# LockedFlysher/optimal_control_problem

Hardware: AMD Instinct MI355X
Metric: QP solves/sec (batched OSQP-ADMM, N=20) (higher is better)
Workload: dtype f64

## Files before the change

optimal_control_problem_amd/csrc/kernel_oc_split.hpp:

```cpp
#pragma once

constexpr int OC_PENDING = 100, OC_PENDING_NONCVX = 101;
template <int NW>
struct OcLds {
  double *X, *Q, *R, *Z, *Y, *W, *RB, *RED;
  int *octab, *co;
};
template <int NW, bool SETUP = false>
__device__ __forceinline__ OcLds<NW> oc_lds(double *lds, const DevPlan &pl, const DevRes &rs, const DevOc &oc) {
  OcLds<NW> L;
  L.X = lds + rs.stage; L.Q = L.X + pl.npad; L.R = SETUP ? L.Q : L.Q + pl.npad;
  double *rend = L.R + pl.npad + rs.rext;
  L.Z = rend; L.Y = L.Z + (SETUP ? oc.zpad : pl.mpad); L.W = L.Y + (SETUP ? pl.npad : pl.mpad);
  L.RB = L.W + pl.mpad; L.RED = L.RB + 16 * NW + 16;
  L.octab = reinterpret_cast<int *>(L.RED + 16 * NW) + 8;
  L.co = L.octab + ((oc.o_pos + 1) & ~1);
  return L;
}
__device__ __forceinline__ int oc_wave_role4(double *lds, int wid, const int lane, const int no_remap) {
  const unsigned hw = __builtin_amdgcn_s_getreg((31 << 11) | 4), la = __builtin_amdgcn_s_getreg((31 << 11) | 6);
  const int simd = (hw >> 4) & 3, slot = (la & 0xff) != 0;
  int *xs = reinterpret_cast<int *>(lds);
  if (lane == 0) xs[wid] = simd;
  bsync<4>();
// ... 65 lines not shown
    cx.rho = uni(io.info[4L * b + 3]);
    cx.c = 1.0; cx.cinv = 1.0;
    const bool okr = factorize_res<NW, (HUB ? 2 : 1), false>(cx, &oc, L.octab, lds);
    if (tid == 0) io.status[b] = okr ? OC_PENDING : OC_PENDING_NONCVX;
    return;
  }
  double c = 1.0;
  int refactor = 1, prev_status = MPCQP_UNSOLVED;
  const bool reuse = REUSE && io.reuse;
  if (reuse) {
    prev_status = io.status[b];
    c = io.cscale[b];
    for (int t = tid; t < npad; t += NT) { if (pl.perm[t] < 0) Qs[t] = 0.0; cx.R[t] = Dg[t]; }
    bsync<NW>();
    for (int j = tid; j < n; j += NT) { const int t = pl.pos[j]; Qs[t] = inq[j] * (c * cx.R[t]); }
    double chg[1] = {0.0};
    for (int i = tid; i < mpad; i += NT) {
      const double ei = Eg[i];
      const double nl = i < m ? ei * fmax(inl[i], -Q_INFTY) : 0.0, nu = i < m ? ei * fmin(inu[i], Q_INFTY) : 0.0;
      if (i < m) {
        const double ol = lb[i], ou = ub[i];
        const int oc_ = (ol < -Q_INFTY * Q_MIN_SCALING && ou > Q_INFTY * Q_MIN_SCALING) ? 0 : (ou - ol < Q_RHO_TOL ? 2 : 1);
        const int nc = (nl < -Q_INFTY * Q_MIN_SCALING && nu > Q_INFTY * Q_MIN_SCALING) ? 0 : (nu - nl < Q_RHO_TOL ? 2 : 1);
        if (oc_ != nc) chg[0] = 1.0;
      }
      lb[i] = nl; ub[i] = nu;
    }
    block_combine<NW, 1, 0>(chg, cx.RED, wid, lane);
    refactor = chg[0] != 0.0;
    c = uni(c); cx.c = c; cx.cinv = uni(1.0 / c);
    bsync<NW>();
  } else {
    const bool a_lds = oc.a_lds, p_lds = oc.p_lds;
    auto scale_phase = [&](double *sA, double *sP, auto iA, auto iP) __attribute__((always_inline)) {
    auto gather8 = [&](const int *__restrict__ src, const double *__restrict__ in, double *dst, const long entries) __attribute__((always_inline)) {
      long e = tid;
      for (; e + 7L * NT < entries; e += 8L * NT) {
        int sr[8]; double v[8];
#pragma unroll
        for (int u = 0; u < 8; u++) sr[u] = src[e + (long)u * NT];
#pragma unroll
        for (int u = 0; u < 8; u++) v[u] = in[max(sr[u], 0)];
#pragma unroll
        for (int u = 0; u < 8; u++) dst[e + (long)u * NT] = sr[u] >= 0 ? v[u] : 0.0;
      }
      for (; e < entries; e += NT) { const int sr = src[e]; dst[e] = sr >= 0 ? in[sr] : 0.0; }
    };
    gather8(pl.A.src, inA, sA, pl.A.entries);
    gather8(pl.P.src, inP, sP, pl.P.entries);
    if constexpr (sizeof(*iA) == 2) { for (long e = tid; e < pl.A.entries; e += NT) iA[e] = (unsigned short)pl.A.idx[e]; }
    if constexpr (sizeof(*iP) == 2) { for (long e = tid; e < pl.P.entries; e += NT) iP[e] = (unsigned short)pl.P.idx[e]; }
    for (int t = tid; t < npad; t += NT) { if (pl.perm[t] < 0) Qs[t] = 0.0; cx.R[t] = 1.0; cx.X[t] = 0.0; }
    for (int i = tid; i < mpad; i += NT) cx.W[i] = 1.0;
    bsync<NW>();
    for (int j = tid; j < n; j += NT) Qs[pl.pos[j]] = inq[j];
    bsync<NW>();
    TS(0);
    c = 1.0;
    double *nPv = cx.Y;
    if (st.scaling > 0) { for (int ch = wid; ch < pl.P.nchunks; ch += NW) { const int t = ch * WAVE + lane; const double x = ell_chunk_mx(sP, iP, cx.R, cx.coP[ch], cx.coP[ch + 1], lane); if (t < npad) nPv[t] = x; } }
    const int shA = pl.P.nchunks % NW;
    auto cost_scale = [&]() {
      double r0 = cx.RED[0], r1 = cx.RED[1];
      for (int w = 1; w < NW; w++) { r0 = fmax(r0, cx.RED[2 * w]); r1 = r1 + cx.RED[2 * w + 1]; }
      c *= 1.0 / limit_scaling(fmax(r1 / (double)n, limit_scaling(r0)));
    };
    for (int it = 0; it < st.scaling; it++) {
      RZ_T0;
      for (int ch = (wid + NW - shA) % NW; ch < pl.A.nchunks; ch += NW) {
        const int i = ch * WAVE + lane;
        const double ei = i < mpad ? cx.W[i] : 0.0;
        const double v = ell_chunk_rc(sA, iA, cx.R, ei, cx.X, cx.coA[ch], cx.coA[ch + 1], lane);
        if (i < mpad) cx.W[i] = ei * (1.0 / sqrt(limit_scaling(ei * v)));
      }
      RZ_T(4);
      bsync<NW>();
      RZ_T(5);
      if (it > 0) cost_scale();
      for (int t = tid; t < npad; t += NT) {
        const double dj = cx.R[t];
        cx.R[t] = dj * (1.0 / sqrt(limit_scaling(fmax(c * dj * nPv[t], dj * cx.X[t]))));
        cx.X[t] = 0.0;
      }
      bsync<NW>();
      RZ_T(6);
      double v[2] = {0.0, 0.0};
      for (int ch = wid; ch < pl.P.nchunks; ch += NW) {
        const int t = ch * WAVE + lane;
        const double x = ell_chunk_mx(sP, iP, cx.R, cx.coP[ch], cx.coP[ch + 1], lane);
        if (t < npad) { nPv[t] = x; v[1] += c * cx.R[t] * x; v[0] = fmax(v[0], fabs(c * cx.R[t] * Qs[t])); }
      }
      v[0] = wave_max(v[0]); v[1] = wave_sum(v[1]);
      if (lane == 0) { cx.RED[2 * wid] = v[0]; cx.RED[2 * wid + 1] = v[1]; }
      RZ_T(7);
    }
    if (st.scaling > 0) { bsync<NW>(); cost_scale(); bsync<NW>(); }
    c = uni(c); cx.c = c; cx.cinv = uni(1.0 / c);
    TS(1);
    for (int ch = wid; ch < pl.A.nchunks; ch += NW) {
      const int i = ch * WAVE + lane; const double ei = i < mpad ? cx.W[i] : 0.0;
      ell_map_chunk<false>(sA, pl.A.idx, nullptr, pl.A.idx, valA, cx.coA[ch], cx.coA[ch + 1], lane, [&](double v, int j) { return v * (ei * cx.R[j]); });
    }
    for (int ch = wid; ch < pl.At.nchunks; ch += NW) {
      const int t = ch * WAVE + lane; const double dj = t < npad ? cx.R[t] : 0.0;
      ell_map_chunk<true>(valAt, pl.At.src, inA, pl.At.idx, valAt, cx.coAt[ch], cx.coAt[ch + 1], lane, [&](double v, int i) { return v * (dj * cx.W[i]); });
      ell_map_chunk<false>(sP, pl.P.idx, nullptr, pl.P.idx, valP, cx.coP[ch], cx.coP[ch + 1], lane, [&](double v, int k) { return v * (c * dj * cx.R[k]); });
    }
    if (oc.tl.on) {
      const DevTile &tl = oc.tl;
      double *tiles = ws + tl.o_tile, *valAr = ws + tl.o_ellAr, *valAtr = ws + tl.o_ellAtr;
      for (long e = tid; e < (long)tl.ntile * BLK; e += NT) {
        const int sidx = tl.tsrc[e];
        double v = 0.0;
        if (sidx >= 0) {
          const int t = (int)(e >> 8), r = (int)(e >> 4) & 15, cc = (int)e & 15;
          v = inA[sidx] * (cx.W[tl.rowid[t * BS + r]] * cx.R[BS * tl.tJ[t] + cc]);
        }
        tiles[e] = v;
      }
      for (int ch = wid; ch < tl.nAr; ch += NW) {
        const int i = ch * WAVE + lane; const double ei = i < mpad ? cx.W[i] : 0.0;
        ell_map_chunk<true>(valAr, tl.Ar_src, inA, tl.Ar_idx, valAr, tl.Ar_off[ch], tl.Ar_off[ch + 1], lane, [&](double v, int j) { return v * (ei * cx.R[j]); });
      }
      for (int ch = wid; ch < tl.nAtr; ch += NW) {
        const int t = ch * WAVE + lane; const double dj = t < npad ? cx.R[t] : 0.0;
        ell_map_chunk<true>(valAtr, tl.Atr_src, inA, tl.Atr_idx, valAtr, tl.Atr_off[ch], tl.Atr_off[ch + 1], lane, [&](double v, int i) { return v * (dj * cx.W[i]); });
      }
    }
    bsync<NW>();
    for (int t = tid; t < npad; t += NT) { Qs[t] *= c * cx.R[t]; Dg[t] = cx.R[t]; }
    for (int i = tid; i < mpad; i += NT) {
      const double ei = cx.W[i];
      Eg[i] = ei;
      lb[i] = i < m ? ei * fmax(inl[i], -Q_INFTY) : 0.0;
      ub[i] = i < m ? ei * fmin(inu[i], Q_INFTY) : 0.0;
    }
    };
    unsigned short *iA16 = reinterpret_cast<unsigned short *>(lds) + oc.ixo_a, *iP16 = reinterpret_cast<unsigned short *>(lds) + oc.ixo_p;
    if (a_lds && p_lds && oc.ix16 == 3) scale_phase(lds, lds + pl.A.entries, iA16, iP16);
    else if (a_lds && p_lds && oc.ix16 == 1) scale_phase(lds, lds + pl.A.entries, iA16, pl.P.idx);
    else if (a_lds && p_lds) scale_phase(lds, lds + pl.A.entries, pl.A.idx, pl.P.idx);
    else if (a_lds) scale_phase(lds, valP, pl.A.idx, pl.P.idx);
    else if (oc.ix16 == 3) scale_phase(valA, valP, iA16, iP16);
    else if (oc.ix16 == 1) scale_phase(valA, valP, iA16, pl.P.idx);
    else scale_phase(valA, valP, pl.A.idx, pl.P.idx);
  }
  bsync<NW>();
  cx.rho = uni(reuse ? io.info[4L * b + 3] : fmin(fmax(io.rho0 && io.rho0[b] > 0.0 ? io.rho0[b] : st.rho, Q_RHO_MIN), Q_RHO_MAX));
  TS(2);
  bool ok = !(reuse && prev_status == MPCQP_NON_CVX);
  if (ok && refactor) ok = factorize_res<NW, (HUB ? 2 : 1), false>(cx, &oc, L.octab, lds);
  if (tid == 0) {
    io.status[b] = ok ? MPCQP_UNSOLVED : MPCQP_NON_CVX; io.iters[b] = 0;
    io.info[4L * b + 3] = cx.rho;
    io.cscale[b] = c;
  }
  TS(3);
#ifdef MPCQP_TIMING
  ts_acc[12] = cx.fts[0]; ts_acc[13] = cx.fts[1]; ts_acc[14] = cx.fts[2]; ts_acc[15] = cx.fts[3];
#ifdef MPCQP_TIMING_RUIZ
  ts_acc[9] = rzacc[0]; ts_acc[10] = rzacc[1]; ts_acc[11] = rzacc[2]; ts_acc[12] = rzacc[3]; ts_acc[13] = rzacc[4];
#endif
#endif
  TS_STORE(io.dbg);
}

template <int NW, int OCG, int OCH, int RF, bool TL, bool PAIRS>
__device__ __forceinline__ void oc_admm_one(const DevPlan &pl, const DevRes &rs, const mpcqp_settings &st, const DevIO &io, const DevOc &oc, double *lds, const int b, const int wid, const int lane) {
  constexpr int NT = NW * WAVE;
  [[maybe_unused]] constexpr int OCU = NW == 4 ? 16 : 8;
  constexpr bool HUB = OCH > 0;
  const int tid = wid * WAVE + lane;
  const OcLds<NW> L = oc_lds<NW>(lds, pl, rs, oc);
  RCtx cx;
  cx.pl = &pl; cx.rs = &rs; cx.st = &st; cx.wid = wid; cx.lane = lane;
  cx.fts[0] = cx.fts[1] = cx.fts[2] = cx.fts[3] = 0;
  double *ws = io.ws + (long)b * pl.ws_stride; cx.ws = ws;
  cx.BL = ws + pl.o_Lf; cx.TMP = lds;
// ... 317 lines not shown
```

optimal_control_problem_amd/csrc/kernel_onchip.hpp:

```cpp
#pragma once

struct DevTile {
  int on, ntile;
  int nAr, nAtr;
  const int *Ar_off, *Ar_idx, *Ar_src, *Atr_off, *Atr_idx, *Atr_src;
  long Ar_entries, Atr_entries;
  const int *tJ, *rowid, *tsrc;
  const int *ta_info, *ta_cnt;
  const unsigned long long *ta_mask;
  const int *tt_info;
  long o_tile, o_ellAr, o_ellAtr;
};
struct DevOc {
  int nbc, has_hub, junc, npw, nhr, nlds, ntab;
  int o_chainE, o_chainF, o_pos, o_fill, ghub_slot, ghub_src;
  const int *a_assign;
  int npair, o_pair;
  int nfill, o_s, o_dbl, ndbl, o_pp;
  int at_poll, at_free;
  int a_lds, p_lds;
  const int *tab;
  const int *asm_rec;
  DevTile tl;
  int resume;
  int ixo_a, ixo_p;
  int ix16, zpad;
};

__host__ __device__ __forceinline__ int oc_swz(int r, int c) {
  return ((r ^ ((r >> 2) & 1)) << 4) | (c ^ (((r >> 1) & 3) << 2) ^ (((r >> 3) & 1) << 1));
}

typedef double d2 __attribute__((ext_vector_type(2)));

struct OcLane {
  unsigned f4;
  unsigned t4;
  int k4;
  int o4;
};
__device__ __forceinline__ OcLane oc_lane(int lane) {
  OcLane ln;
  const int n = lane & 15, kk = lane >> 4;
  ln.f4 = 0; ln.t4 = 0;
#pragma unroll
  for (int K = 0; K < 4; K++) { ln.f4 |= (unsigned)oc_swz(n, kk + 4 * K) << (8 * K); ln.t4 |= (unsigned)oc_swz(kk + 4 * K, n) << (8 * K); }
  ln.k4 = kk; ln.o4 = 4 * ((lane >> 2) & 3) + (lane >> 4);
  return ln;
}
__device__ __forceinline__ d4 oc_mv(const d4 a, const d4 v, d4 acc) {
  acc = __builtin_amdgcn_mfma_f64_16x16x4f64(a[0], v[0], acc, 0, 0, 0);
  acc = __builtin_amdgcn_mfma_f64_16x16x4f64(a[1], v[1], acc, 0, 0, 0);
  acc = __builtin_amdgcn_mfma_f64_16x16x4f64(a[2], v[2], acc, 0, 0, 0);
  acc = __builtin_amdgcn_mfma_f64_16x16x4f64(a[3], v[3], acc, 0, 0, 0);
  return acc;
}
__device__ __forceinline__ double oc_mv4(const double a, const double v, const double acc) { return __builtin_amdgcn_mfma_f64_4x4x4f64(a, v, acc, 0, 0, 0); }
__device__ __forceinline__ d4 oc_ld4(const double *blk, const unsigned pk) { return d4{blk[pk & 255], blk[(pk >> 8) & 255], blk[(pk >> 16) & 255], blk[pk >> 24]}; }
__device__ __forceinline__ d4 oc_ldF4(const double *blk, const OcLane &ln) { return oc_ld4(blk, ln.f4); }
// ... 794 lines not shown
```

optimal_control_problem_amd/csrc/kernel_resident.hpp:

```cpp
#pragma once

#ifdef MPCQP_TIMING
#define TS_DECL unsigned long long ts_last = __builtin_amdgcn_s_memtime(), ts_acc[16] = {0}; const unsigned long long ts_first = ts_last, ts_rt0 = __builtin_amdgcn_s_memrealtime()
#define TS(k) do { unsigned long long t_ = __builtin_amdgcn_s_memtime(); ts_acc[k] += t_ - ts_last; ts_last = t_; } while (0)
#define TS_STORE(ptr) do { if (tid == 0 && (ptr)) { for (int k_ = 0; k_ < 16; k_++) (ptr)[16L * b + k_] = (long long)ts_acc[k_]; \
    if (b == 0) { (ptr)[16L * gridDim.x + 126] = (long long)(__builtin_amdgcn_s_memtime() - ts_first); (ptr)[16L * gridDim.x + 127] = (long long)(__builtin_amdgcn_s_memrealtime() - ts_rt0); } } } while (0)
#else
#define TS_DECL
#ifdef MPCQP_ASM_MARKS
#define TS(k) do { __builtin_amdgcn_sched_barrier(0); asm volatile("; TS " #k ::: "memory"); } while (0)
#else
#define TS(k) __builtin_amdgcn_sched_barrier(0)
#endif
#define TS_STORE(ptr)
#endif
struct DevRes {
  int nphase, ntemp, nconst, rext;
  const int *lv_ptr, *lv_diag, *lw_ptr, *lw_slot, *lw_g, *lu_ptr, *lu_dst, *lu_tmp, *lu_b, *g_ptr, *g_seg;
  int n_seg, nlev; long stage;
  int tmp_alias;
};


struct RCtx {
// ... 112 lines not shown
  double acc = 0.0;
  int u0 = 0;
  for (; u0 + 8 <= w; u0 += 8) acc = ell_batch_rc<8>(val, idx, din, ei, colacc, e0, u0, r0, w, acc);
  if ((w - u0) & 4) { acc = ell_batch_rc<4>(val, idx, din, ei, colacc, e0, u0, r0, w, acc); u0 += 4; }
  if ((w - u0) & 2) { acc = ell_batch_rc<2>(val, idx, din, ei, colacc, e0, u0, r0, w, acc); u0 += 2; }
  if ((w - u0) & 1) acc = ell_batch_rc<1>(val, idx, din, ei, colacc, e0, u0, r0, w, acc);
  return acc;
}
template <int U, class IT>
__device__ __forceinline__ double ell_batch_mx(const double *__restrict__ &vp, const IT *__restrict__ &ip, const double *in, double acc) {
  double v[U], x[U]; int ix[U];
#pragma unroll
  for (int u = 0; u < U; u++) { v[u] = vp[u * WAVE]; ix[u] = ip[u * WAVE]; }
#pragma unroll
  for (int u = 0; u < U; u++) x[u] = in[ix[u]];
  asm volatile("" ::: "memory");
#pragma unroll
  for (int u = 0; u < U; u++) acc = fmax(acc, fabs(v[u]) * x[u]);
  vp += U * WAVE; ip += U * WAVE;
  return acc;
}
template <class IT>
__device__ __forceinline__ double ell_chunk_mx(const double *__restrict__ val, const IT *__restrict__ idx, const double *in, const int s0, const int s1, const int lane) {
  const double *__restrict__ vp = val + ((long)s0 * WAVE + lane);
  const IT *__restrict__ ip = idx + ((long)s0 * WAVE + lane);
  double acc = 0.0;
  int rem = s1 - s0;
  for (; rem >= 8; rem -= 8) acc = ell_batch_mx<8>(vp, ip, in, acc);
  if (rem & 4) acc = ell_batch_mx<4>(vp, ip, in, acc);
  if (rem & 2) acc = ell_batch_mx<2>(vp, ip, in, acc);
  if (rem & 1) acc = ell_batch_mx<1>(vp, ip, in, acc);
  return acc;
}
template <bool INDIRECT, int U, class F>
__device__ __forceinline__ void ell_map_batch(const double *&vp, const int *__restrict__ &sp, const double *in, const int *__restrict__ &ip, double *&op, F &f) {
  double v[U]; int ix[U], sr[U];
#pragma unroll
  for (int u = 0; u < U; u++) { if (INDIRECT) sr[u] = sp[u * WAVE]; else v[u] = vp[u * WAVE]; ix[u] = ip[u * WAVE]; }
  if (INDIRECT) {
#pragma unroll
    for (int u = 0; u < U; u++) v[u] = sr[u] >= 0 ? in[sr[u]] : 0.0;
  }
#pragma unroll
  for (int u = 0; u < U; u++) op[u * WAVE] = f(v[u], ix[u]);
  if (INDIRECT) sp += U * WAVE; else vp += U * WAVE;
  ip += U * WAVE; op += U * WAVE;
}
template <bool INDIRECT, class F>
__device__ __forceinline__ void ell_map_chunk(const double *val, const int *__restrict__ src, const double *in, const int *__restrict__ idx, double *out,
                                              const int s0, const int s1, const int lane, F &&f) {
  const long o = (long)s0 * WAVE + lane;
  const double *vp = val + o; const int *__restrict__ sp = src + o; const int *__restrict__ ip = idx + o; double *op = out + o;
  int rem = s1 - s0;
  for (; rem >= 8; rem -= 8) ell_map_batch<INDIRECT, 8>(vp, sp, in, ip, op, f);
  if (rem & 4) ell_map_batch<INDIRECT, 4>(vp, sp, in, ip, op, f);
  if (rem & 2) ell_map_batch<INDIRECT, 2>(vp, sp, in, ip, op, f);
  if (rem & 1) ell_map_batch<INDIRECT, 1>(vp, sp, in, ip, op, f);
}
template <int NW, int UMAX = 16, class F>
__device__ __forceinline__ void ell_rows_w(const DevEll &E, const int *co, const double *__restrict__ val, const double *in, int wid, int lane, F &&f) {
  for (int c = wid; c < E.nchunks; c += NW) f(c * WAVE + lane, ell_chunk<false, UMAX>(val, E.idx, in, co[c], co[c + 1], lane));
}
template <int NW, class F>
__device__ __forceinline__ void ell_rowmax_w(const DevEll &E, const int *co, const double *__restrict__ val, const double *in, int wid, int lane, F &&f) {
  for (int c = wid; c < E.nchunks; c += NW) f(c * WAVE + lane, ell_chunk<true>(val, E.idx, in, co[c], co[c + 1], lane));
}
// ... 904 lines not shown
```

optimal_control_problem_amd/csrc/mpcqp.hip:

```cpp
#include <map>
#include <mutex>
#include "kernels_all.hpp"
#include "kernels_util.hpp"
#include "reduced.hpp"

static_assert(SEL_ERR_ARG == MPCQP_ERR_ARG && SEL_ERR_LIMIT == MPCQP_ERR_LIMIT, "select.hpp reports its refusals in the codes of include/mpcqp.h");

static thread_local std::string g_last_error;
static int fail(int code, const std::string &msg) { g_last_error = msg; return code; }
int mpcqp_set_error(int code, const std::string &msg) { return fail(code, msg); }
int mpcqp_pick_device(int requested, int *device) {
  int ndev = 0;
  if (hipGetDeviceCount(&ndev) != hipSuccess || ndev <= 0) return fail(MPCQP_ERR_NO_GPU, "hipGetDeviceCount found no device");
  int dev = requested;
  if (dev < 0) { if (hipGetDevice(&dev) != hipSuccess) dev = 0; }
  if (dev >= ndev) return fail(MPCQP_ERR_ARG, "device ordinal out of range");
  hipDeviceProp_t prop;
  if (hipGetDeviceProperties(&prop, dev) != hipSuccess) return fail(MPCQP_ERR_HIP, "hipGetDeviceProperties failed");
  if (std::string(prop.gcnArchName).find("gfx950") == std::string::npos)
    return fail(MPCQP_ERR_NO_GPU, std::string("device is ") + prop.gcnArchName + ", kernels are built for gfx950 only");
  *device = dev;
  return MPCQP_OK;
}
#define HIPCHK(expr)                                                                              \
// ... 230 lines not shown
        std::copy(rec, rec + 4, ai.begin() + 32 * (size_t)c + 4 * u);
      }
    }
    UP(upload(h, ai, &t.ta_info)); UP(upload(h, ac, &t.ta_cnt));
    std::vector<int> ti(16 * (size_t)pl.At.nchunks, 0);
    for (int J = 0; J < 4 * pl.At.nchunks; J++) {
      const int tt = (J < pl.nb && tp.tt_ptr[J + 1] > tp.tt_ptr[J]) ? tp.tt_tid[tp.tt_ptr[J]] : tp.ntile;
      int rec[4] = {tt, first(tt), rows(tt), 0};
      std::copy(rec, rec + 4, ti.begin() + 4 * (size_t)J);
    }
    UP(upload(h, ti, &t.tt_info));
  }
  std::vector<unsigned long long> mask(pl.A.nchunks, 0ull);
  for (size_t k = 0; k < (size_t)tp.ntile * BS; k++) if (tp.rowid[k] >= 0) mask[tp.rowid[k] / WAVE] |= 1ull << (tp.rowid[k] % WAVE);
  UP(upload(h, mask, &t.ta_mask));
  t.o_tile = s.wl.tile; t.o_ellAr = s.wl.ellAr; t.o_ellAtr = s.wl.ellAtr;
  return MPCQP_OK;
}
static int upload_onchip(mpcqp_handle *h, int cus) {
  Selection &s = h->sel; const Plan &pl = s.plan; const OcPlan &o = s.ocplan; const ResPlan &rp = s.rplan; DevRes &dr = h->dres; DevOc &d = h->doc;
  dr.stage = s.stage; dr.rext = oc_rext(rp.nw, std::max<int>(1, (int)o.pairs.size())); dr.nconst = 0; dr.n_seg = 0;
  d.nbc = o.nbc; d.has_hub = o.has_hub; d.junc = o.junc; d.npw = o.npw; d.nhr = o.nhr; d.nlds = o.nlds; d.ntab = (int)o.tab.size();
  d.o_chainE = o.o_chainE; d.o_chainF = o.o_chainF; d.o_pos = o.o_pos; d.o_fill = o.o_fill; d.ghub_slot = o.ghub_slot; d.ghub_src = o.ghub_src;
  d.npair = (int)o.pairs.size(); d.o_pair = o.o_pair; d.nfill = o.nfill; d.o_s = o.o_s; d.o_dbl = o.o_dbl; d.ndbl = (int)o.dbl.size(); d.o_pp = o.o_pp;
  d.at_poll = s.at_poll; d.at_free = s.at_free;
  d.a_lds = s.a_lds; d.p_lds = s.p_lds;
  if (s.vtiles && !mpcqp_kernel_oc_admm_tl(s.waves, s.oc_ng(), s.oc_nh())) s.vtiles = false;
  UP(upload(h, o.tab, &d.tab));
  UP(upload(h, oc_asm_records(pl), &d.asm_rec));
  if (s.tiles || s.vtiles) UP(upload_tiles(h));
  const SetupShape &su = s.setup; DevRes &ds = h->dres_setup; DevOc &dd = h->doc_setup;
  ds = dr; dd = d;
  dd.a_lds = su.a_lds; dd.p_lds = su.p_lds; dd.ix16 = su.ix16; dd.zpad = su.zpad; dd.ixo_a = su.ixo_a; dd.ixo_p = su.ixo_p;
  ds.stage = su.stage;
  if (!s.split) return MPCQP_OK;
  if (s.oc8 && !s.vtiles && !s.a_assign.empty()) UP(upload(h, s.a_assign, &d.a_assign));
  if (s.oc8) {
    int nb = 0; h->qslots = 256;
    if (hipOccupancyMaxActiveBlocksPerMultiprocessor(&nb, oc_admm_of(h, false), s.waves * WAVE, (size_t)s.lds) == hipSuccess && nb > 0) {
      h->qslots = nb * (cus > 0 ? cus : 256);
    } else (void)hipGetLastError();
    UP(dalloc(h, &h->qctr, 16 * 16));
  }
  if (h->knobs.verbose) fprintf(stderr, "%s, %d resident workgroups\n", setup_shape_text(s).c_str(), h->qslots);
  return MPCQP_OK;
}
static int alloc_workspace(mpcqp_handle *h) {
  const size_t stride = (size_t)h->sel.wl.stride, batch = (size_t)h->batch; const int n = h->n, m = h->m;
  UP(dalloc(h, &h->ws, stride * batch));
  HIPCHK(hipMemset(h->ws, 0, stride * batch * sizeof(double))); HIPCHK(hipStreamSynchronize(0));
  UP(dalloc(h, &h->ox, batch * n)); UP(dalloc(h, &h->oy, batch * std::max(m, 1))); UP(dalloc(h, &h->oz, batch * std::max(m, 1)));
  UP(dalloc(h, &h->oinfo, batch * 4)); UP(dalloc(h, &h->ocs, batch));
  UP(dalloc(h, &h->ostatus, batch)); UP(dalloc(h, &h->oiters, batch));
#ifdef MPCQP_TIMING
  UP(dalloc(h, &h->odbg, batch * 16 + 128));
#endif
  UP(dalloc(h, &h->order[0], batch)); UP(dalloc(h, &h->order[1], batch));
  return MPCQP_OK;
}
#undef UP
static int prepare_kernels(mpcqp_handle *h) {
  const Selection &s = h->sel;
  if (s.lds > 48 * 1024) {
    static std::mutex mu; static std::map<std::pair<const void *, int>, long> limit;
    const void *fns[4] = {res_kernel_of(h, false), res_kernel_of(h, true), nullptr, nullptr};
    if (s.waves == 0) fns[0] = fns[1] = s.stream_pd8 ? (const void *)mpcqp_admm_kernel<8> : (const void *)mpcqp_admm_kernel<4>;
// ... 635 lines not shown
```

optimal_control_problem_amd/csrc/plan.hpp:

```cpp
#pragma once
#include <algorithm>
#include <cstdint>
#include <map>
#include <set>
#include <string>
#include <utility>
#include <vector>

namespace mpcqp {

constexpr int BS = 16;
constexpr int BLK = BS * BS;
constexpr int WAVE = 64;

struct Ell {
  int nrows = 0, nchunks = 0;
  std::vector<int> chunk_off;
  std::vector<int> idx;
  std::vector<int> src;
  std::vector<int> flag;
  int slots() const { return chunk_off.empty() ? 0 : chunk_off.back(); }
  long entries() const { return (long)slots() * WAVE; }
};

struct EllEntry { int idx, src, flag; };

inline int ell_batches8(int w) { int r = w % 8; return w / 8 + (r & 1) + ((r >> 1) & 1) + ((r >> 2) & 1); }
inline Ell build_ell(const std::vector<std::vector<EllEntry>> &rows, int pad4 = 0) {
  Ell e;
  e.nrows = (int)rows.size();
  e.nchunks = (e.nrows + WAVE - 1) / WAVE;
  e.chunk_off.assign(e.nchunks + 1, 0);
  for (int c = 0; c < e.nchunks; c++) {
    size_t w = 0;
    for (int r = c * WAVE; r < std::min(e.nrows, (c + 1) * WAVE); r++) w = std::max(w, rows[r].size());
    if (pad4 == 1 && w > 2) w = (w + 3) / 4 * 4;
    if (pad4 == 2 && w > 2) { size_t best = w; for (size_t w2 = w + 1; w2 <= w + 3; w2++) if (ell_batches8((int)w2) < ell_batches8((int)best)) best = w2; w = best; }
    e.chunk_off[c + 1] = e.chunk_off[c] + (int)w;
  }
  e.idx.assign(e.entries(), 0); e.src.assign(e.entries(), -1); e.flag.assign(e.entries(), 0);
  for (int r = 0; r < e.nrows; r++) {
    int c = r / WAVE, lane = r % WAVE;
    for (size_t s = 0; s < rows[r].size(); s++) {
      long p = ((long)e.chunk_off[c] + (long)s) * WAVE + lane;
      e.idx[p] = rows[r][s].idx; e.src[p] = rows[r][s].src; e.flag[p] = rows[r][s].flag;
    }
  }
  return e;
}

enum { OP_DIAG = 0, OP_OFF = 1 };
inline int pack_op(int kind, int src, int dst) { return kind | (src << 1) | (dst << 16); }

enum { FAC_SUB = 0, FAC_POTRF = 1, FAC_TRSM = 2 };
struct FacOp { int type, dst, a, b; };

struct Plan {
  int n = 0, m = 0, npad = 0, mpad = 0, nb = 0;
  int nnzP_in = 0, nnzA_in = 0, nnzP_triu = 0;
  int ordering = 0;
  std::vector<int> pos;
  std::vector<int> perm;
  std::vector<int> singleton;
  Ell A, At, P;
  int nblk = 0;
  std::vector<int> blkI, blkJ;
  std::vector<int> fwd_ops, bwd_ops;
  std::vector<int> bwd_of;
  std::vector<FacOp> fac;
  int nT = 0;
  std::vector<int> tpos;
  std::vector<int> asm_ptr;
  std::vector<int> asm_a, asm_b;
  std::vector<int> asm_pidx;
  std::vector<int> blk_diag;
  std::vector<std::vector<int>> colrows;
  std::string error;
};

enum { SOP_SUB = 0, SOP_SUBT = 1, SOP_SET = 2 };
inline int pack_sop(int kind, int slot, int src, int dst) { return kind | (slot << 2) | (src << 14) | (dst << 23); }
// ... 857 lines not shown
```

optimal_control_problem_amd/csrc/select.hpp:

```cpp
#pragma once
#include <climits>
#include <cstdio>
#include <cstdlib>
#include <string>
#include <vector>

#include "plan.hpp"

namespace mpcqp {

constexpr int OC_NG = 5, OC_NH = 3;
struct Oc8Inst { int ng, nh; bool zyg; };
constexpr Oc8Inst OC8_INST[2] = {{4, 4, false}, {7, 7, false}};
constexpr long OC_LDS_MAX = 80 * 1024;
constexpr long OC8_LDS_MAX = 160 * 1024;
constexpr int OC8_MAX_CHAIN = 64;
constexpr long LDS_MAX = 160 * 1024;

constexpr int SEL_ERR_ARG = 1, SEL_ERR_LIMIT = 5;

struct Knobs {
  bool variant_named = false; std::string variant;
  bool autotune = false;
  bool verbose = false;
  bool no_lpt = false;
  bool no_twist = false;
  bool no_oc = false;
  bool no_oc8 = false;
  bool no_res2 = false;
  bool no_dissect = false;
  bool no_padtwist = false;
  bool oc_mono = false;
  bool oc_pad4 = false;
  bool no_zyg = false;
  bool gb_occ2 = false;
  bool gb_occ3 = false;
  bool no_res1x = false;
  bool no_res3 = false;
  bool pd4 = false;
  long lds_min = 0;
  int tiles = 0;
  int vtiles = 0;
  int doubles = -1;
  bool late = false;
  int resume_rounds = 1;
  bool no_ix16 = false;
  long setup_cap = LONG_MIN;
  bool no_abalance = false;
  bool no_touch = false;
  bool touch4 = false;
  bool touch8 = false;
  bool no_remap = false;
  int pipe_streams = 2;

  static Knobs from_env() {
    auto set = [](const char *name) { return getenv(name) != nullptr; };
    auto one = [](const char *name) { const char *e = getenv(name); return !e ? 0 : e[0] == '1' ? 2 : 1; };
    Knobs k;
    if (const char *e = getenv("MPCQP_VARIANT")) { k.variant_named = true; k.variant = e; }
    k.autotune = one("MPCQP_AUTOTUNE") == 2;
    k.verbose = set("MPCQP_VERBOSE");
    k.no_lpt = set("MPCQP_NO_LPT");
    k.no_twist = set("MPCQP_NO_TWIST");
    k.no_oc = set("MPCQP_NO_OC");
    k.no_oc8 = set("MPCQP_NO_OC8");
    k.no_res2 = set("MPCQP_NO_RES2");
    k.no_dissect = set("MPCQP_NO_DISSECT");
    k.no_padtwist = set("MPCQP_NO_PADTWIST");
    k.oc_mono = set("MPCQP_OC_MONO");
    k.oc_pad4 = set("MPCQP_OC_PAD4");
    k.no_zyg = set("MPCQP_NO_ZYG");
    k.gb_occ2 = set("MPCQP_GB_OCC2");
    k.gb_occ3 = set("MPCQP_GB_OCC3");
    k.no_res1x = set("MPCQP_NO_RES1X");
    k.no_res3 = set("MPCQP_NO_RES3");
    k.pd4 = set("MPCQP_PD4");
    if (const char *e = getenv("MPCQP_LDS_MIN")) k.lds_min = atol(e);
    k.tiles = one("MPCQP_TILES");
    k.vtiles = one("MPCQP_VTILES");
    if (const char *e = getenv("MPCQP_DOUBLES")) k.doubles = std::max(0, atoi(e));
    k.late = set("MPCQP_LATE");
    if (const char *e = getenv("MPCQP_RESUME_ROUNDS")) k.resume_rounds = std::max(0, std::min(atoi(e), 8));
    k.no_ix16 = set("MPCQP_NO_IX16");
    if (const char *e = getenv("MPCQP_SETUP_CAP")) k.setup_cap = atol(e);
    k.no_abalance = set("MPCQP_NO_ABALANCE");
    k.no_touch = set("MPCQP_NO_TOUCH");
    k.touch4 = set("MPCQP_TOUCH4");
    k.touch8 = set("MPCQP_TOUCH8");
    k.no_remap = set("MPCQP_NO_REMAP");
    if (const char *e = getenv("MPCQP_PIPE_STREAMS")) k.pipe_streams = std::max(1, std::min(atoi(e), 8));
    return k;
  }
};

struct SetupShape {
  int nw = 0; long lds = 0, stage = 0;
  int a_lds = 0, p_lds = 0, ix16 = 0, zpad = 0, ixo_a = 0, ixo_p = 0;
  long vecs = 0, tabw = 0;
};

struct Selection {
  int err = 0; std::string error;
  int waves = 0;
  bool wide = false;
  bool gblocks = false;
  bool zyg = false;
  bool occ3 = false;
  bool occ4 = false;
  bool res1x = false;
  int res3 = 0;
  bool stream_pd8 = false;
  bool oc = false;
  int oc8 = 0;
  bool split = false;
  bool tiles = false;
  bool vtiles = false;
// ... 310 lines not shown
```

Before: 1.064 million.

## Keep Ruiz-scaling A/P matrix slices in registers when LDS staging is unavailable

When A or P cannot be staged in LDS, the Ruiz equilibration loop re-reads the ELL values and indices from global memory on every iteration. Each wave now loads its few A and P chunks, with packed 16-bit indices, into registers once, then runs the column/row max passes and the final P scaling write from registers. A global P slab gather is skipped when every wave's P chunks fit. This raises register pressure and adds a second code path. It is gated by size limits and an env knob.

```diff
diff --git a/optimal_control_problem_amd/csrc/kernel_oc_split.hpp b/optimal_control_problem_amd/csrc/kernel_oc_split.hpp
--- a/optimal_control_problem_amd/csrc/kernel_oc_split.hpp
+++ b/optimal_control_problem_amd/csrc/kernel_oc_split.hpp
@@ -121,7 +121,20 @@
     bsync<NW>();
   } else {
     const bool a_lds = oc.a_lds, p_lds = oc.p_lds;
-    auto scale_phase = [&](double *sA, double *sP, auto iA, auto iP) __attribute__((always_inline)) {
+    auto scale_phase = [&](double *sA, double *sP, auto iA, auto iP, auto rg) __attribute__((always_inline)) {
+    constexpr bool RG = decltype(rg)::value;
+    const int shA = pl.P.nchunks % NW, firstA = (wid + NW - shA) % NW;
+    [[maybe_unused]] unsigned aR[RZ_CAPA], pI[RZ_CAPP / 2]; [[maybe_unused]] double pV[RZ_CAPP], qs[RZ_KP];
+    [[maybe_unused]] RzList<RZ_KA> LA; [[maybe_unused]] RzList<RZ_KP> LP;
+    bool ra = false, rp = false, p_slab = true;
+    if constexpr (RG) {
+      const bool on = !oc.no_ruiz_regs && pl.A.entries <= 65536 && npad <= 65536 && mpad <= 65536;
+      LA = rz_list<NW, RZ_KA, RZ_CAPA>(pl.A.chunk_off, pl.A.nchunks, firstA); LP = rz_list<NW, RZ_KP, RZ_CAPP>(pl.P.chunk_off, pl.P.nchunks, wid);
+      ra = on && LA.fits; rp = on && LP.fits;
+      bool every = on;
+      for (int w = 0; w < NW; w++) every = every && rz_list<NW, RZ_KP, RZ_CAPP>(pl.P.chunk_off, pl.P.nchunks, w).fits;
+      p_slab = !every;
+    }
     auto gather8 = [&](const int *__restrict__ src, const double *__restrict__ in, double *dst, const long entries) __attribute__((always_inline)) {
       long e = tid;
       for (; e + 7L * NT < entries; e += 8L * NT) {
@@ -136,7 +149,7 @@
       for (; e < entries; e += NT) { const int sr = src[e]; dst[e] = sr >= 0 ? in[sr] : 0.0; }
     };
     gather8(pl.A.src, inA, sA, pl.A.entries);
-    gather8(pl.P.src, inP, sP, pl.P.entries);
+    if (p_slab) gather8(pl.P.src, inP, sP, pl.P.entries);
     if constexpr (sizeof(*iA) == 2) { for (long e = tid; e < pl.A.entries; e += NT) iA[e] = (unsigned short)pl.A.idx[e]; }
     if constexpr (sizeof(*iP) == 2) { for (long e = tid; e < pl.P.entries; e += NT) iP[e] = (unsigned short)pl.P.idx[e]; }
     for (int t = tid; t < npad; t += NT) { if (pl.perm[t] < 0) Qs[t] = 0.0; cx.R[t] = 1.0; cx.X[t] = 0.0; }
@@ -144,11 +157,28 @@
     bsync<NW>();
     for (int j = tid; j < n; j += NT) Qs[pl.pos[j]] = inq[j];
     bsync<NW>();
+    if constexpr (RG) {
+      if (ra) rz_fill_a(LA, iA, lane, aR);
+      if (rp) {
+        rz_fill_p(LP, iP, pl.P.src, inP, lane, pV, pI);
+#pragma unroll
+        for (int q = 0; q < RZ_KP; q++) { const int t = (wid + q * NW) * WAVE + lane; qs[q] = (q < LP.nk && t < npad) ? Qs[t] : 0.0; }
+      }
+    }
     TS(0);
     c = 1.0;
     double *nPv = cx.Y;
-    if (st.scaling > 0) { for (int ch = wid; ch < pl.P.nchunks; ch += NW) { const int t = ch * WAVE + lane; const double x = ell_chunk_mx(sP, iP, cx.R, cx.coP[ch], cx.coP[ch + 1], lane); if (t < npad) nPv[t] = x; } }
-    const int shA = pl.P.nchunks % NW;
+    if (st.scaling > 0) {
+      if (RG && rp) {
+        if constexpr (RG) {
+          double xs[RZ_KP];
+          rz_pass_p(LP, pV, pI, cx.R, xs);
+#pragma unroll
+          for (int q = 0; q < RZ_KP; q++) { const int t = (wid + q * NW) * WAVE + lane; if (q < LP.nk && t < npad) nPv[t] = xs[q]; }
+        }
+      } else
+      for (int ch = wid; ch < pl.P.nchunks; ch += NW) { const int t = ch * WAVE + lane; const double x = ell_chunk_mx(sP, iP, cx.R, cx.coP[ch], cx.coP[ch + 1], lane); if (t < npad) nPv[t] = x; }
+    }
     auto cost_scale = [&]() {
       double r0 = cx.RED[0], r1 = cx.RED[1];
       for (int w = 1; w < NW; w++) { r0 = fmax(r0, cx.RED[2 * w]); r1 = r1 + cx.RED[2 * w + 1]; }
@@ -156,7 +186,10 @@
     };
     for (int it = 0; it < st.scaling; it++) {
       RZ_T0;
-      for (int ch = (wid + NW - shA) % NW; ch < pl.A.nchunks; ch += NW) {
+      if (RG && ra) {
+        if constexpr (RG) rz_pass_a<NW>(LA, aR, sA, cx.R, cx.X, cx.W, firstA, mpad, lane);
+      } else
+      for (int ch = firstA; ch < pl.A.nchunks; ch += NW) {
         const int i = ch * WAVE + lane;
         const double ei = i < mpad ? cx.W[i] : 0.0;
         const double v = ell_chunk_rc(sA, iA, cx.R, ei, cx.X, cx.coA[ch], cx.coA[ch + 1], lane);
@@ -174,6 +207,17 @@
       bsync<NW>();
       RZ_T(6);
       double v[2] = {0.0, 0.0};
+      if (RG && rp) {
+        if constexpr (RG) {
+          double xs[RZ_KP];
+          rz_pass_p(LP, pV, pI, cx.R, xs);
+#pragma unroll
+          for (int q = 0; q < RZ_KP; q++) {
+            const int t = (wid + q * NW) * WAVE + lane; const double x = xs[q];
+            if (q < LP.nk && t < npad) { nPv[t] = x; v[1] += c * cx.R[t] * x; v[0] = fmax(v[0], fabs(c * cx.R[t] * qs[q])); }
+          }
+        }
+      } else
       for (int ch = wid; ch < pl.P.nchunks; ch += NW) {
         const int t = ch * WAVE + lane;
         const double x = ell_chunk_mx(sP, iP, cx.R, cx.coP[ch], cx.coP[ch + 1], lane);
@@ -186,6 +230,7 @@
     if (st.scaling > 0) { bsync<NW>(); cost_scale(); bsync<NW>(); }
     c = uni(c); cx.c = c; cx.cinv = uni(1.0 / c);
     TS(1);
+    if constexpr (RG) { if (rp) rz_write_p<NW>(LP, pV, pI, cx.R, valP, c, wid, npad, lane); }
     for (int ch = wid; ch < pl.A.nchunks; ch += NW) {
       const int i = ch * WAVE + lane; const double ei = i < mpad ? cx.W[i] : 0.0;
       ell_map_chunk<false>(sA, pl.A.idx, nullptr, pl.A.idx, valA, cx.coA[ch], cx.coA[ch + 1], lane, [&](double v, int j) { return v * (ei * cx.R[j]); });
@@ -193,7 +238,7 @@
     for (int ch = wid; ch < pl.At.nchunks; ch += NW) {
       const int t = ch * WAVE + lane; const double dj = t < npad ? cx.R[t] : 0.0;
       ell_map_chunk<true>(valAt, pl.At.src, inA, pl.At.idx, valAt, cx.coAt[ch], cx.coAt[ch + 1], lane, [&](double v, int i) { return v * (dj * cx.W[i]); });
-      ell_map_chunk<false>(sP, pl.P.idx, nullptr, pl.P.idx, valP, cx.coP[ch], cx.coP[ch + 1], lane, [&](double v, int k) { return v * (c * dj * cx.R[k]); });
+      if (!(RG && rp)) ell_map_chunk<false>(sP, pl.P.idx, nullptr, pl.P.idx, valP, cx.coP[ch], cx.coP[ch + 1], lane, [&](double v, int k) { return v * (c * dj * cx.R[k]); });
     }
     if (oc.tl.on) {
       const DevTile &tl = oc.tl;
@@ -226,13 +271,14 @@
     }
     };
     unsigned short *iA16 = reinterpret_cast<unsigned short *>(lds) + oc.ixo_a, *iP16 = reinterpret_cast<unsigned short *>(lds) + oc.ixo_p;
-    if (a_lds && p_lds && oc.ix16 == 3) scale_phase(lds, lds + pl.A.entries, iA16, iP16);
-    else if (a_lds && p_lds && oc.ix16 == 1) scale_phase(lds, lds + pl.A.entries, iA16, pl.P.idx);
-    else if (a_lds && p_lds) scale_phase(lds, lds + pl.A.entries, pl.A.idx, pl.P.idx);
-    else if (a_lds) scale_phase(lds, valP, pl.A.idx, pl.P.idx);
-    else if (oc.ix16 == 3) scale_phase(valA, valP, iA16, iP16);
-    else if (oc.ix16 == 1) scale_phase(valA, valP, iA16, pl.P.idx);
-    else scale_phase(valA, valP, pl.A.idx, pl.P.idx);
+    constexpr std::false_type plain{}; constexpr std::true_type regs{};
+    if (a_lds && p_lds && oc.ix16 == 3) scale_phase(lds, lds + pl.A.entries, iA16, iP16, plain);
+    else if (a_lds && p_lds && oc.ix16 == 1) scale_phase(lds, lds + pl.A.entries, iA16, pl.P.idx, plain);
+    else if (a_lds && p_lds) scale_phase(lds, lds + pl.A.entries, pl.A.idx, pl.P.idx, plain);
+    else if (a_lds) scale_phase(lds, valP, pl.A.idx, pl.P.idx, regs);
+    else if (oc.ix16 == 3) scale_phase(valA, valP, iA16, iP16, regs);
+    else if (oc.ix16 == 1) scale_phase(valA, valP, iA16, pl.P.idx, regs);
+    else scale_phase(valA, valP, pl.A.idx, pl.P.idx, regs);
   }
   bsync<NW>();
   cx.rho = uni(reuse ? io.info[4L * b + 3] : fmin(fmax(io.rho0 && io.rho0[b] > 0.0 ? io.rho0[b] : st.rho, Q_RHO_MIN), Q_RHO_MAX));
diff --git a/optimal_control_problem_amd/csrc/kernel_onchip.hpp b/optimal_control_problem_amd/csrc/kernel_onchip.hpp
--- a/optimal_control_problem_amd/csrc/kernel_onchip.hpp
+++ b/optimal_control_problem_amd/csrc/kernel_onchip.hpp
@@ -25,6 +25,7 @@
   int resume;
   int ixo_a, ixo_p;
   int ix16, zpad;
+  int no_ruiz_regs = 0;
 };
 
 __host__ __device__ __forceinline__ int oc_swz(int r, int c) {
diff --git a/optimal_control_problem_amd/csrc/kernel_resident.hpp b/optimal_control_problem_amd/csrc/kernel_resident.hpp
--- a/optimal_control_problem_amd/csrc/kernel_resident.hpp
+++ b/optimal_control_problem_amd/csrc/kernel_resident.hpp
@@ -168,6 +168,171 @@
   if (rem & 1) acc = ell_batch_mx<1>(vp, ip, in, acc);
   return acc;
 }
+constexpr int RZ_U = 4;
+constexpr int RZ_KA = RUIZ_REG_CHUNKS_A, RZ_KP = RUIZ_REG_CHUNKS_P, RZ_CAPA = RUIZ_REG_SLOTS_A, RZ_CAPP = RUIZ_REG_SLOTS_P;
+static_assert(RZ_CAPA % RZ_U == 0 && RZ_CAPP % RZ_U == 0 && RZ_CAPP % 2 == 0, "register slot capacities: whole batches, index pairs");
+template <int K> struct RzList { int nk, tot, fits, s0, s1, s2, e0, e1, e2; };
+static_assert(RUIZ_REG_CHUNKS_A <= 3 && RUIZ_REG_CHUNKS_P <= 3, "RzList holds three chunks");
+__device__ __forceinline__ int rz_pick3(const int a, const int b, const int c, const int k) { return __builtin_amdgcn_readfirstlane(k == 0 ? a : k == 1 ? b : c); }
+template <int K> __device__ __forceinline__ int rz_end(const RzList<K> &L, const int k) { const int a = L.e0, b = L.e1, c = K < 3 ? b : L.e2; return rz_pick3(a, b, c, k); }
+template <int K> __device__ __forceinline__ int rz_s0(const RzList<K> &L, const int k) { const int a = L.s0, b = L.s1, c = K < 3 ? b : L.s2; return rz_pick3(a, b, c, k); }
+template <int K>
+__device__ __forceinline__ void rz_put(double (&a)[K], const int k, const double v) {
+#pragma unroll
+  for (int q = 0; q < K; q++) a[q] = k == q ? v : a[q];
+}
+template <int NW, int K, int CAP>
+__device__ __forceinline__ RzList<K> rz_list(const int *__restrict__ chunk_off, const int nchunks, const int first) {
+  RzList<K> L; L.nk = 0; L.tot = 0;
+  auto one = [&](const int q, int &s0, int &end) {
+    const int ch = first + q * NW; const bool in = q < K && ch < nchunks;
+    const int a = __builtin_amdgcn_readfirstlane(in ? chunk_off[ch] : 0), b = __builtin_amdgcn_readfirstlane(in ? chunk_off[ch + 1] : 0);
+    s0 = a; L.tot += b - a; end = L.tot; L.nk += in;
+  };
+  one(0, L.s0, L.e0); one(1, L.s1, L.e1); one(2, L.s2, L.e2);
+  L.fits = first + K * NW >= nchunks && L.tot <= CAP;
+  return L;
+}
+struct RzWalk { int k, beg, w, s0; };
+template <int K>
+__device__ __forceinline__ RzWalk rz_walk0(const RzList<K> &L) { return RzWalk{0, 0, L.e0, L.s0}; }
+template <int K>
+__device__ __forceinline__ bool rz_step(const RzList<K> &L, RzWalk &wk, const int u) {
+  bool moved = false;
+  while (u == wk.beg + wk.w) { wk.k++; wk.beg += wk.w; wk.w = rz_end(L, wk.k) - wk.beg; wk.s0 = rz_s0(L, wk.k); moved = true; }
+  return moved;
+}
+template <class IT>
+__device__ __forceinline__ void rz_fill_a(const RzList<RZ_KA> &L, const IT *__restrict__ idx, const int lane, unsigned (&aR)[RZ_CAPA]) {
+  RzWalk wk = rz_walk0(L);
+  int r0 = wk.w > 0 ? lane % wk.w : 0;
+#pragma unroll
+  for (int g = 0; g < RZ_CAPA / RZ_U; g++) {
+    unsigned ai[RZ_U];
+#pragma unroll
+    for (int j = 0; j < RZ_U; j++) {
+      const int u = g * RZ_U + j;
+      aR[u] = (unsigned)lane; ai[j] = 0;
+      if (u < L.tot) {
+        if (rz_step(L, wk, u)) r0 = lane % wk.w;
+        int su = u - wk.beg + r0; su -= su >= wk.w ? wk.w : 0;
+        const int e = (wk.s0 + su) * WAVE + lane;
+        aR[u] = (unsigned)e; ai[j] = (unsigned)idx[e];
+      }
+    }
+#pragma unroll
+    for (int j = 0; j < RZ_U; j++) aR[g * RZ_U + j] |= ai[j] << 16;
+  }
+}
+__device__ __forceinline__ int rz_pidx(const unsigned (&pI)[RZ_CAPP / 2], const int u) { return (u & 1) ? (int)(pI[u >> 1] >> 16) : (int)(pI[u >> 1] & 0xffffu); }
+__device__ __forceinline__ unsigned rz_opaque(unsigned r) { asm volatile("" : "+v"(r)); return r; }
+template <class IT>
+__device__ __forceinline__ void rz_fill_p(const RzList<RZ_KP> &L, const IT *__restrict__ idx, const int *__restrict__ src, const double *__restrict__ in, const int lane,
+                                          double (&pV)[RZ_CAPP], unsigned (&pI)[RZ_CAPP / 2]) {
+  RzWalk wk = rz_walk0(L);
+#pragma unroll
+  for (int g = 0; g < RZ_CAPP / RZ_U; g++) {
+    int sr[RZ_U]; unsigned ix[RZ_U];
+#pragma unroll
+    for (int j = 0; j < RZ_U; j++) {
+      const int u = g * RZ_U + j;
+      sr[j] = -1; ix[j] = 0;
+      if (u < L.tot) {
+        rz_step(L, wk, u);
+        const int e = (wk.s0 + u - wk.beg) * WAVE + lane;
+        sr[j] = src[e]; ix[j] = (unsigned)idx[e];
+      }
+    }
+#pragma unroll
+    for (int j = 0; j < RZ_U; j++) pV[g * RZ_U + j] = in[max(sr[j], 0)];
+#pragma unroll
+    for (int j = 0; j < RZ_U; j++) { const int u = g * RZ_U + j; pV[u] = sr[j] >= 0 ? pV[u] : 0.0; }
+#pragma unroll
+    for (int j = 0; j < RZ_U; j += 2) pI[(g * RZ_U + j) >> 1] = ix[j] | (ix[j + 1] << 16);
+  }
+}
+template <int NW>
+__device__ __forceinline__ void rz_pass_a(const RzList<RZ_KA> &L, const unsigned (&aR)[RZ_CAPA], const double *__restrict__ val, const double *din, double *colacc, double *W,
+                                          const int first, const int mpad, const int lane) {
+  auto e_of = [&](const int k) { const int i = (first + k * NW) * WAVE + lane; return (k < L.nk && i < mpad) ? W[i] : 0.0; };
+  double accs[RZ_KA];
+#pragma unroll
+  for (int q = 0; q < RZ_KA; q++) accs[q] = 0.0;
+  int k = 0, nxt = L.e0;
+  double acc = 0.0, ei = e_of(0);
+#pragma unroll
+  for (int g = 0; g < RZ_CAPA / RZ_U; g++) {
+    if (g * RZ_U < L.tot) {
+      double v[RZ_U], x[RZ_U]; unsigned ix[RZ_U];
+#pragma unroll
+      for (int j = 0; j < RZ_U; j++) { const unsigned r = rz_opaque(aR[g * RZ_U + j]); ix[j] = r >> 16; v[j] = fabs(val[r & 0xffffu]); x[j] = din[ix[j]]; }
+      asm volatile("" ::: "memory");
+#pragma unroll
+      for (int j = 0; j < RZ_U; j++) {
+        const int u = g * RZ_U + j;
+        if (u < L.tot) {
+          while (u == nxt) { rz_put(accs, k, acc); k++; acc = 0.0; ei = e_of(k); nxt = rz_end(L, k); }
+          acc = fmax(acc, v[j] * x[j]);
+          if (v[j] != 0.0) __hip_atomic_fetch_max((lds_u64 *)(colacc + ix[j]), (unsigned long long)__double_as_longlong(v[j] * ei), __ATOMIC_RELAXED, __HIP_MEMORY_SCOPE_WORKGROUP);
+        }
+      }
+    }
+  }
+  rz_put(accs, k, acc);
+#pragma unroll
+  for (int q = 0; q < RZ_KA; q++) {
+    const int i = (first + q * NW) * WAVE + lane;
+    if (q < L.nk && i < mpad) { const double e = W[i]; W[i] = e * (1.0 / sqrt(limit_scaling(e * accs[q]))); }
+  }
+}
+__device__ __forceinline__ void rz_pass_p(const RzList<RZ_KP> &L, const double (&pV)[RZ_CAPP], const unsigned (&pI)[RZ_CAPP / 2], const double *in, double (&out)[RZ_KP]) {
+#pragma unroll
+  for (int q = 0; q < RZ_KP; q++) out[q] = 0.0;
+  int k = 0, nxt = L.e0;
+  double acc = 0.0;
+#pragma unroll
+  for (int g = 0; g < RZ_CAPP / RZ_U; g++) {
+    if (g * RZ_U < L.tot) {
+      double x[RZ_U];
+#pragma unroll
+      for (int j = 0; j < RZ_U; j += 2) { const unsigned r = rz_opaque(pI[(g * RZ_U + j) >> 1]); x[j] = in[r & 0xffffu]; x[j + 1] = in[r >> 16]; }
+      asm volatile("" ::: "memory");
+#pragma unroll
+      for (int j = 0; j < RZ_U; j++) {
+        const int u = g * RZ_U + j;
+        if (u < L.tot) {
+          while (u == nxt) { rz_put(out, k, acc); k++; acc = 0.0; nxt = rz_end(L, k); }
+          acc = fmax(acc, fabs(pV[u]) * x[j]);
+        }
+      }
+    }
+  }
+  rz_put(out, k, acc);
+}
+template <int NW>
+__device__ __forceinline__ void rz_write_p(const RzList<RZ_KP> &L, const double (&pV)[RZ_CAPP], const unsigned (&pI)[RZ_CAPP / 2], const double *D, double *out, const double c,
+                                           const int first, const int npad, const int lane) {
+  auto d_of = [&](const int k) { const int t = (first + k * NW) * WAVE + lane; return (k < L.nk && t < npad) ? D[t] : 0.0; };
+  RzWalk wk = rz_walk0(L);
+  double dj = d_of(0);
+#pragma unroll
+  for (int g = 0; g < RZ_CAPP / RZ_U; g++) {
+    if (g * RZ_U < L.tot) {
+      double x[RZ_U];
+#pragma unroll
+      for (int j = 0; j < RZ_U; j++) x[j] = D[rz_pidx(pI, g * RZ_U + j)];
+#pragma unroll
+      for (int j = 0; j < RZ_U; j++) {
+        const int u = g * RZ_U + j;
+        if (u < L.tot) {
+          if (rz_step(L, wk, u)) dj = d_of(wk.k);
+          out[(long)(wk.s0 + u - wk.beg) * WAVE + lane] = pV[u] * (c * dj * x[j]);
+        }
+      }
+    }
+  }
+}
+
 template <bool INDIRECT, int U, class F>
 __device__ __forceinline__ void ell_map_batch(const double *&vp, const int *__restrict__ &sp, const double *in, const int *__restrict__ &ip, double *&op, F &f) {
   double v[U]; int ix[U], sr[U];
diff --git a/optimal_control_problem_amd/csrc/mpcqp.hip b/optimal_control_problem_amd/csrc/mpcqp.hip
--- a/optimal_control_problem_amd/csrc/mpcqp.hip
+++ b/optimal_control_problem_amd/csrc/mpcqp.hip
@@ -286,6 +286,7 @@
   const SetupShape &su = s.setup; DevRes &ds = h->dres_setup; DevOc &dd = h->doc_setup;
   ds = dr; dd = d;
   dd.a_lds = su.a_lds; dd.p_lds = su.p_lds; dd.ix16 = su.ix16; dd.zpad = su.zpad; dd.ixo_a = su.ixo_a; dd.ixo_p = su.ixo_p;
+  dd.no_ruiz_regs = h->knobs.no_ruiz_regs ? 1 : 0;
   ds.stage = su.stage;
   if (!s.split) return MPCQP_OK;
   if (s.oc8 && !s.vtiles && !s.a_assign.empty()) UP(upload(h, s.a_assign, &d.a_assign));
diff --git a/optimal_control_problem_amd/csrc/plan.hpp b/optimal_control_problem_amd/csrc/plan.hpp
--- a/optimal_control_problem_amd/csrc/plan.hpp
+++ b/optimal_control_problem_amd/csrc/plan.hpp
@@ -47,6 +47,13 @@
     }
   }
   return e;
+}
+
+constexpr int RUIZ_REG_CHUNKS_A = 3, RUIZ_REG_SLOTS_A = 20, RUIZ_REG_CHUNKS_P = 2, RUIZ_REG_SLOTS_P = 24;
+inline bool ruiz_regs_fit(const std::vector<int> &chunk_off, int nchunks, int first, int nw, int max_chunks, int max_slots) {
+  int tot = 0;
+  for (int q = 0, ch = first; q < max_chunks && ch < nchunks; q++, ch += nw) tot += chunk_off[ch + 1] - chunk_off[ch];
+  return first + max_chunks * nw >= nchunks && tot <= max_slots;
 }
 
 enum { OP_DIAG = 0, OP_OFF = 1 };
diff --git a/optimal_control_problem_amd/csrc/select.hpp b/optimal_control_problem_amd/csrc/select.hpp
--- a/optimal_control_problem_amd/csrc/select.hpp
+++ b/optimal_control_problem_amd/csrc/select.hpp
@@ -45,6 +45,7 @@
   bool late = false;
   int resume_rounds = 1;
   bool no_ix16 = false;
+  bool no_ruiz_regs = false;
   long setup_cap = LONG_MIN;
   bool no_abalance = false;
   bool no_touch = false;
@@ -82,6 +83,7 @@
     k.late = set("MPCQP_LATE");
     if (const char *e = getenv("MPCQP_RESUME_ROUNDS")) k.resume_rounds = std::max(0, std::min(atoi(e), 8));
     k.no_ix16 = set("MPCQP_NO_IX16");
+    k.no_ruiz_regs = one("MPCQP_NO_RUIZ_REGS") == 2;
     if (const char *e = getenv("MPCQP_SETUP_CAP")) k.setup_cap = atol(e);
     k.no_abalance = set("MPCQP_NO_ABALANCE");
     k.no_touch = set("MPCQP_NO_TOUCH");
```

New measurement: 1.089 million (median of 6 runs). 2.3% higher.
